# dblanm/gnn-manip

Measured on AMD Instinct MI355X. Metric: rollout steps/sec (N particles, 10 MP steps, hidden=128), higher is better.
Workload: dtype f32; 1 GPU; north_star target: N=100k dense synthetic scene, conn_r=0.015, max_neighbours=20, hidden=128, 10 MP steps; n_particles=100000, hidden=128, edges_last_step=1966056, k_steps=6, candidates_per_gpu=1, parallelism=candidate-parallel x1

## Files before the change

### gnn_manip_amd/csrc/common.h

```cpp
#pragma once
#include <hip/hip_runtime.h>
#include <stdint.h>
#include <stdio.h>
#include <string.h>
#include <mutex>
#include "../../include/gnn_manip_hip.h"

namespace gm {

void set_error(const char* fmt, ...);

#define GM_HIP_CHECK(expr)                                                                  \
    do {                                                                                    \
        hipError_t _e = (expr);                                                             \
        if (_e != hipSuccess) {                                                             \
            gm::set_error("%s failed: %s (%s:%d)", #expr, hipGetErrorString(_e), __FILE__,  \
                          __LINE__);                                                        \
            return GM_ERR_HIP;                                                              \
        }                                                                                   \
    } while (0)

#define GM_REQUIRE(cond, code, ...)          \
    do {                                     \
        if (!(cond)) {                       \
// ... 57 lines not shown
    }
    size_t used() const { return align_up(off, 256); }
};

enum : int { ERRF_NONFINITE_POS = 1, ERRF_BAD_EDGE_INDEX = 2, ERRF_CAPACITY = 4, ERRF_SPLIT_RANGE = 8 };

struct GraphHeader {
    int n_edges;
    int error_flags;
    int ncells;
    int dims[3];
    unsigned bbox_min[3];
    unsigned bbox_max[3];
    double origin[3];
    double inv_h;
    int n_per_graph;
    int ncells_local;
    int ticket;
    int order_skip;
};

struct GraphWs {
    GraphHeader* hdr;
    int* cell_of;
    int* cell_start;
    int* cell_cursor;
    float4* sorted;
    int* cnt;
    int* out_ptr;
    int* nbr;
    int* scan_cells;
    int* scan_cnt;
    int max_cells;
    size_t bytes;
};
int max_cells_for(int64_t n);
GraphWs carve_graph(void* ws, int64_t n, int max_nb);

struct CsrHeader {
    int n_edges;
    int error_flags;
    int flow;
    int pad;
};
struct CsrWs {
    CsrHeader* hdr;
    int* in_ptr;
    int* cursor;
    int* dst;
    int* src;
    int* eid;
    int* scan_in;
    int* sort_tmp;
    int64_t cap;
    int* blocks;
    size_t bytes;
};
CsrWs carve_csr(void* ws, int64_t n, int64_t cap);

enum ProfKind : int { PROF_EDGE = 0, PROF_NODE = 1, PROF_GRAPH = 2, PROF_ENC = 3, PROF_REST = 4, PROF_KINDS = 5 };
constexpr int PROF_MAX = 4096;
struct ProfState {
    int mask = 0;
    int count[PROF_KINDS] = {};
    int dropped[PROF_KINDS] = {};
    hipEvent_t* start[PROF_KINDS] = {};
    hipEvent_t* stop[PROF_KINDS] = {};
    ~ProfState();
};
struct ProfScope {
    ProfState* p;
    int idx;
    int kind;
    hipStream_t s;
    ProfScope(ProfState* state, int kind, hipStream_t s);
    ~ProfScope();
};

struct StepClear;
int rollout_pre_features(float* obs, int64_t n, const gm_feature_desc* d, const int* rank, const float* target, float* out,
                         hipStream_t s, const StepClear* clear);
int rollout_integrate_post(float* obs, int64_t n, const gm_feature_desc* d, const float* pred, const int* rank,
                           const float* target, float* pred_out, hipStream_t s);
int renumber_gather(const float* in, float* out, int k, int64_t n, int D, const int* perm, const void* graph_ws, const int* total_in,
                    int* total_out, const int* rank_caller, int* rank_out, hipStream_t s);
int renumber_scatter(const float* in, float* out, int frames, int64_t n, int D, const int* total, hipStream_t s);
int csr_from_graph_with_features(const void* graph_ws, int64_t n, int K, void* csr_ws, size_t csr_ws_bytes, const float* pos,
                                 int64_t pos_stride, float conn_r, float* edge_attr, int flow, hipStream_t s);
int csr_from_edge_index(const int64_t* ei, int64_t n, int64_t e, int flow, void* csr_ws, size_t csr_ws_bytes, bool with_blocks, hipStream_t stream);

int cell_order(const float* pos, int64_t pos_stride, int64_t n, int64_t n_per, double conn_r, int K, void* graph_ws, size_t graph_ws_bytes,
               int* perm, hipStream_t s);

size_t scan_state_ints(int64_t n_max);
struct ScanJob {
    const int* in;
    int* out;
    long long n;
    int* total_out;
    int* state;
};
int scan_lookback(const ScanJob* jobs, int n_jobs, hipStream_t s);

struct ClearJob {
    int* p;
    long long n;
    int v;
};
constexpr int kClearJobsMax = 12;
struct GraphHeader;
struct StepClear {
    int n_jobs = 0;
    ClearJob job[kClearJobsMax] = {};
    GraphHeader* gh = nullptr;
    CsrHeader* ch = nullptr;
    int flow = 0;
    int add(int* p, long long n, int v) {
        if (!p || n <= 0) return GM_OK;
        GM_REQUIRE(n_jobs < kClearJobsMax, GM_ERR_INVALID_ARGUMENT, "StepClear: more than %d resets in one pass", kClearJobsMax);
        job[n_jobs++] = ClearJob{p, n, v};
        return GM_OK;
    }
};
int launch_step_clear(const StepClear& c, hipStream_t s);
#if defined(__HIPCC__)
__device__ inline void step_clear_run(const StepClear& c, long long t, long long nt) {
    for (int q = 0; q < c.n_jobs; ++q) {
        int* p = c.job[q].p;
        const long long n = c.job[q].n;
        const int v = c.job[q].v;
        if ((reinterpret_cast<uintptr_t>(p) & 15) == 0 && n >= 4) {
            const long long n4 = n >> 2;
            int4* p4 = reinterpret_cast<int4*>(p);
            for (long long i = t; i < n4; i += nt) p4[i] = make_int4(v, v, v, v);
            for (long long i = (n4 << 2) + t; i < n; i += nt) p[i] = v;
        } else {
            for (long long i = t; i < n; i += nt) p[i] = v;
        }
    }
    if (t == 0) {
        if (GraphHeader* hdr = c.gh) {
            hdr->n_edges = 0;
            hdr->error_flags = 0;
            hdr->ncells = 1;
            for (int a = 0; a < 3; ++a) {
                hdr->bbox_min[a] = 0xffffffffu;
                hdr->bbox_max[a] = 0u;
                hdr->dims[a] = 1;
                hdr->origin[a] = 0.0;
            }
            hdr->inv_h = 1.0;
            hdr->n_per_graph = 1;
            hdr->ncells_local = 1;
            hdr->ticket = 0;
            hdr->order_skip = 0;
        }
        if (CsrHeader* ch = c.ch) {
            ch->n_edges = 0;
            ch->error_flags = 0;
            ch->flow = c.flow;
            ch->pad = 0;
        }
    }
}
#endif
struct GraphWs;
// ... 11 lines not shown
```

### gnn_manip_amd/csrc/features.hip

```cpp
#include "common.h"

namespace gm {

struct FeatParams {
    int k, D, cart, mat, ctrl;
    float r;
    float vm[3], vs[3], am[3], as[3], lo[3], hi[3];
};

static int to_params(const gm_feature_desc* d, FeatParams* p, const char* who) {
    GM_REQUIRE(d != nullptr, GM_ERR_INVALID_ARGUMENT, "%s: null feature descriptor", who);
    GM_REQUIRE(d->k_steps >= 2 && d->k_steps <= 64, GM_ERR_INVALID_ARGUMENT, "%s: k_steps=%d out of range", who, d->k_steps);
    GM_REQUIRE(d->data_dim >= 4 && d->cart_col >= 0 && d->cart_col + 3 <= d->data_dim, GM_ERR_INVALID_ARGUMENT,
               "%s: bad cartesian columns", who);
    GM_REQUIRE(d->material_col >= 0 && d->material_col < d->data_dim, GM_ERR_INVALID_ARGUMENT, "%s: bad material column", who);
    GM_REQUIRE(d->control_col < 0 || d->control_col + 3 <= d->data_dim, GM_ERR_INVALID_ARGUMENT, "%s: bad control columns", who);
    GM_REQUIRE(d->conn_r > 0.0, GM_ERR_INVALID_ARGUMENT, "%s: conn_r must be > 0", who);
    p->k = d->k_steps; p->D = d->data_dim; p->cart = d->cart_col; p->mat = d->material_col; p->ctrl = d->control_col;
    p->r = (float)d->conn_r;
    for (int a = 0; a < 3; ++a) {
        p->vm[a] = d->vel_mean[a]; p->vs[a] = d->vel_std[a];
        p->am[a] = d->acc_mean[a]; p->as[a] = d->acc_std[a];
        p->lo[a] = d->lower_bounds[a]; p->hi[a] = d->upper_bounds[a];
    }
// ... 1 lines not shown
}

__global__ void __launch_bounds__(256) node_features_kernel(const float* __restrict__ obs, int64_t n, FeatParams P,
                                                             float* __restrict__ out) {
    const int64_t i = (int64_t)blockIdx.x * blockDim.x + threadIdx.x;
    if (i >= n) return;
    const int F = 3 * (P.k - 1) + 7 + (P.ctrl >= 0 ? 3 : 0);
    float* o = out + i * F;
    const int64_t fs = n * P.D;
    const float* row = obs + i * P.D;
    float prev[3], cur[3];
#pragma unroll
    for (int a = 0; a < 3; ++a) prev[a] = row[P.cart + a];
    for (int t = 1; t < P.k; ++t) {
#pragma unroll
        for (int a = 0; a < 3; ++a) {
            cur[a] = row[t * fs + P.cart + a];
            o[(t - 1) * 3 + a] = __fdiv_rn(__fsub_rn(__fsub_rn(cur[a], prev[a]), P.vm[a]), P.vs[a]);
            prev[a] = cur[a];
        }
    }
    float* b = o + 3 * (P.k - 1);
#pragma unroll
    for (int a = 0; a < 3; ++a) {
        float l = __fdiv_rn(__fsub_rn(cur[a], P.lo[a]), P.r);
        float u = __fdiv_rn(__fsub_rn(P.hi[a], cur[a]), P.r);
        b[a] = fminf(fmaxf(l, -1.f), 1.f);
        b[3 + a] = fminf(fmaxf(u, -1.f), 1.f);
    }
    const float* last = row + (int64_t)(P.k - 1) * fs;
    b[6] = last[P.mat];
    if (P.ctrl >= 0) {
#pragma unroll
        for (int a = 0; a < 3; ++a) b[7 + a] = __fdiv_rn(__fsub_rn(last[P.ctrl + a], P.vm[a]), P.vs[a]);
    }
}

__device__ __forceinline__ void edge_feat(const float* __restrict__ pos, int64_t stride, int64_t s, int64_t r, float cr,
                                          float* __restrict__ o) {
    float d[3];
#pragma unroll
    for (int a = 0; a < 3; ++a) d[a] = __fdiv_rn(__fsub_rn(pos[s * stride + a], pos[r * stride + a]), cr);
    float q = __fmul_rn(d[0], d[0]);
    q = __fadd_rn(q, __fmul_rn(d[1], d[1]));
    q = __fadd_rn(q, __fmul_rn(d[2], d[2]));
    *reinterpret_cast<float4*>(o) = make_float4(d[0], d[1], d[2], __fsqrt_rn(q));
}

__global__ void __launch_bounds__(256) edge_features_kernel(const float* __restrict__ pos, int64_t stride,
                                                             const int64_t* __restrict__ snd,
                                                             const int64_t* __restrict__ rcv, int64_t e, float cr,
                                                             float* __restrict__ out) {
    const int64_t i = (int64_t)blockIdx.x * blockDim.x + threadIdx.x;
    if (i >= e) return;
    edge_feat(pos, stride, snd[i], rcv[i], cr, out + i * 4);
}

__global__ void __launch_bounds__(256) edge_features_csr_kernel(const float* __restrict__ pos, int64_t stride,
                                                                 const CsrHeader* __restrict__ hdr,
                                                                 const int* __restrict__ src, const int* __restrict__ dst,
                                                                 float cr, float* __restrict__ out) {
    const int e = hdr->n_edges;
    const bool swap = hdr->flow != 0;
    for (int64_t i = (int64_t)blockIdx.x * blockDim.x + threadIdx.x; i < e; i += (int64_t)gridDim.x * blockDim.x)
        edge_feat(pos, stride, swap ? dst[i] : src[i], swap ? src[i] : dst[i], cr, out + i * 4);
}

__global__ void __launch_bounds__(256) integrate_kernel(const float* __restrict__ pred, const float* __restrict__ obs,
                                                         int64_t n, FeatParams P, float* __restrict__ next_pos) {
    const int64_t i = (int64_t)blockIdx.x * blockDim.x + threadIdx.x;
    if (i >= n) return;
    const int64_t fs = n * P.D;
    const float* l1 = obs + (int64_t)(P.k - 1) * fs + i * P.D + P.cart;
    const float* l2 = obs + (int64_t)(P.k - 2) * fs + i * P.D + P.cart;
#pragma unroll
    for (int a = 0; a < 3; ++a) {
        float acc = __fadd_rn(__fmul_rn(pred[i * 3 + a], P.as[a]), P.am[a]);
        float lv = __fsub_rn(l1[a], l2[a]);
        float v = __fadd_rn(lv, acc);
        next_pos[i * 3 + a] = __fadd_rn(l1[a], v);
    }
}

__global__ void __launch_bounds__(256) pre_features_kernel(float* __restrict__ obs, int64_t n, FeatParams P,
                                                            const int* __restrict__ rank, const float* __restrict__ target,
                                                            float* __restrict__ out, StepClear clr) {
    const int64_t i = (int64_t)blockIdx.x * blockDim.x + threadIdx.x;
    step_clear_run(clr, i, (long long)gridDim.x * blockDim.x);
    if (i >= n) return;
    const int64_t fs = n * P.D;
    float* row = obs + i * P.D;
    float* last = row + (int64_t)(P.k - 1) * fs;
    if (rank && P.ctrl >= 0) {
        const int rk = rank[i];
        if (rk >= 0) {
#pragma unroll
            for (int a = 0; a < 3; ++a) {
                const float cur = last[P.cart + a];
                last[P.ctrl + a] = target ? __fsub_rn(target[(int64_t)rk * 3 + a], cur) : cur;
            }
        }
    }
    const int F = 3 * (P.k - 1) + 7 + (P.ctrl >= 0 ? 3 : 0);
    float* o = out + i * F;
    float prev[3], cur[3];
#pragma unroll
    for (int a = 0; a < 3; ++a) prev[a] = row[P.cart + a];
    for (int t = 1; t < P.k; ++t) {
#pragma unroll
        for (int a = 0; a < 3; ++a) {
            cur[a] = row[t * fs + P.cart + a];
            o[(t - 1) * 3 + a] = __fdiv_rn(__fsub_rn(__fsub_rn(cur[a], prev[a]), P.vm[a]), P.vs[a]);
            prev[a] = cur[a];
        }
    }
    float* b = o + 3 * (P.k - 1);
#pragma unroll
    for (int a = 0; a < 3; ++a) {
        float l = __fdiv_rn(__fsub_rn(cur[a], P.lo[a]), P.r);
        float u = __fdiv_rn(__fsub_rn(P.hi[a], cur[a]), P.r);
        b[a] = fminf(fmaxf(l, -1.f), 1.f);
        b[3 + a] = fminf(fmaxf(u, -1.f), 1.f);
    }
    b[6] = last[P.mat];
    if (P.ctrl >= 0) {
#pragma unroll
        for (int a = 0; a < 3; ++a) b[7 + a] = __fdiv_rn(__fsub_rn(last[P.ctrl + a], P.vm[a]), P.vs[a]);
    }
}

__global__ void __launch_bounds__(256) integrate_post_kernel(float* __restrict__ obs, int64_t n, FeatParams P,
                                                              const float* __restrict__ pred, const int* __restrict__ rank,
                                                              const float* __restrict__ target, float* __restrict__ pred_out) {
    const int64_t i = (int64_t)blockIdx.x * blockDim.x + threadIdx.x;
    if (i >= n) return;
    const int64_t fs = n * P.D;
    float* row = obs + i * P.D;
    const float* l1 = row + (int64_t)(P.k - 1) * fs + P.cart;
    const float* l2 = row + (int64_t)(P.k - 2) * fs + P.cart;
    float nxt[3];
#pragma unroll
    for (int a = 0; a < 3; ++a) {
        const float pa = pred[i * 3 + a];
        if (pred_out) pred_out[i * 3 + a] = pa;
        const float acc = __fadd_rn(__fmul_rn(pa, P.as[a]), P.am[a]);
        const float lv = __fsub_rn(l1[a], l2[a]);
        nxt[a] = __fadd_rn(l1[a], __fadd_rn(lv, acc));
    }
    for (int t = 0; t + 1 < P.k; ++t)
        for (int d = 0; d < P.D; ++d) row[t * fs + d] = row[(t + 1) * fs + d];
    float* last = row + (int64_t)(P.k - 1) * fs;
    const int rk = rank ? rank[i] : -1;
    if (rk < 0) {
#pragma unroll
        for (int a = 0; a < 3; ++a) last[P.cart + a] = nxt[a];
    } else if (target) {
#pragma unroll
        for (int a = 0; a < 3; ++a) last[P.cart + a] = target[(int64_t)rk * 3 + a];
    }
}

__global__ void __launch_bounds__(1024) rigid_rank_kernel(const float* __restrict__ obs, int64_t n, FeatParams P,
                                                           int* __restrict__ rank, int* __restrict__ n_rigid) {
    __shared__ int wsum[16];
    __shared__ int carry_s;
    const float* last = obs + (int64_t)(P.k - 1) * n * P.D;
    const int lane = threadIdx.x & 63, wave = threadIdx.x >> 6;
    if (threadIdx.x == 0) carry_s = 0;
    __syncthreads();
    for (int64_t b = 0; b < n; b += 1024) {
        int64_t i = b + threadIdx.x;
        int f = (i < n && last[i * P.D + P.mat] == 1.0f) ? 1 : 0;
        int incl = f;
#pragma unroll
        for (int d = 1; d < 64; d <<= 1) {
            int t = __shfl_up(incl, d, 64);
            if (lane >= d) incl += t;
        }
        if (lane == 63) wsum[wave] = incl;
        __syncthreads();
        int base = carry_s;
        for (int w = 0; w < wave; ++w) base += wsum[w];
        if (i < n) rank[i] = f ? base + incl - 1 : -1;
        __syncthreads();
        if (threadIdx.x == 1023) carry_s = base + incl;
        __syncthreads();
    }
    if (threadIdx.x == 0 && n_rigid) *n_rigid = carry_s;
}

__global__ void __launch_bounds__(256) state_pre_kernel(float* __restrict__ obs, int64_t n, FeatParams P,
                                                         const int* __restrict__ rank, const float* __restrict__ target) {
    const int64_t i = (int64_t)blockIdx.x * blockDim.x + threadIdx.x;
    if (i >= n) return;
    const int rk = rank[i];
    if (rk < 0) return;
    float* last = obs + (int64_t)(P.k - 1) * n * P.D + i * P.D;
#pragma unroll
    for (int a = 0; a < 3; ++a) {
        float cur = last[P.cart + a];
        last[P.ctrl + a] = target ? __fsub_rn(target[(int64_t)rk * 3 + a], cur) : cur;
    }
}

__global__ void __launch_bounds__(256) state_post_kernel(float* __restrict__ obs, int64_t n, FeatParams P,
                                                          const float* __restrict__ next_pos,
                                                          const int* __restrict__ rank, const float* __restrict__ target) {
    const int64_t i = (int64_t)blockIdx.x * blockDim.x + threadIdx.x;
    if (i >= n) return;
    const int64_t fs = n * P.D;
    float* row = obs + i * P.D;
    for (int t = 0; t + 1 < P.k; ++t)
        for (int d = 0; d < P.D; ++d) row[t * fs + d] = row[(t + 1) * fs + d];
    float* last = row + (int64_t)(P.k - 1) * fs;
    const int rk = rank ? rank[i] : -1;
    if (rk < 0) {
#pragma unroll
        for (int a = 0; a < 3; ++a) last[P.cart + a] = next_pos[i * 3 + a];
    } else if (target) {
#pragma unroll
        for (int a = 0; a < 3; ++a) last[P.cart + a] = target[(int64_t)rk * 3 + a];
    }
}

__global__ void __launch_bounds__(256) rigid_transform_kernel(const float* __restrict__ init, int64_t nr,
                                                               const float* __restrict__ cst, int64_t steps, float tx,
                                                               float ty, float tz, float* __restrict__ out) {
    const int64_t id = (int64_t)blockIdx.x * blockDim.x + threadIdx.x;
    if (id >= nr * steps) return;
    const int64_t t = id / nr, i = id - t * nr;
    const float c = cst[t * 3], s = cst[t * 3 + 1], typ = cst[t * 3 + 2];
    const float i0 = __fsub_rn(tx, init[i * 3 + 0]);
    const float i1 = __fsub_rn(ty, init[i * 3 + 2]);
    const float i2 = __fsub_rn(tz, init[i * 3 + 1]);
    const float p0 = __fadd_rn(i0, tx);
    const float p1 = __fadd_rn(__fmaf_rn(-s, i2, __fmul_rn(c, i1)), typ);
    const float p2 = __fadd_rn(__fmaf_rn(c, i2, __fmul_rn(s, i1)), tz);
    out[id * 3 + 0] = p0;
    out[id * 3 + 2] = p1;
    out[id * 3 + 1] = p2;
}

// ... 5 lines not shown
    const float* gt = g + t * nr * 3;
    double dc = 0.0, ds = 0.0, dt = 0.0;
    for (int64_t i = tid; i < nr; i += 256) {
        const double i1 = (double)ty - (double)init[i * 3 + 2];
        const double i2 = (double)tz - (double)init[i * 3 + 1];
        const double g1 = gt[i * 3 + 1], g2 = gt[i * 3 + 2];
        dc += g2 * i1 + g1 * i2;
        ds += g1 * i1 - g2 * i2;
        dt += g2;
    }
    red[0][tid] = dc; red[1][tid] = ds; red[2][tid] = dt;
    __syncthreads();
    for (int w = 128; w >= 1; w >>= 1) {
        if (tid < w) {
#pragma unroll
            for (int a = 0; a < 3; ++a) red[a][tid] += red[a][tid + w];
        }
        __syncthreads();
    }
    if (tid < 3) d_cst[t * 3 + tid] = (float)red[tid][0];
}

__global__ void __launch_bounds__(256) renumber_gather_kernel(const float* __restrict__ in, float* __restrict__ out, int k, int64_t n, int D,
                                                               const int* __restrict__ perm, const GraphHeader* __restrict__ ghdr,
                                                               const int* __restrict__ total_in, int* __restrict__ total_out,
                                                               const int* __restrict__ rank_caller, int* __restrict__ rank_out) {
    const int64_t id = (int64_t)blockIdx.x * blockDim.x + threadIdx.x;
    if (id >= (int64_t)k * n) return;
    const int64_t t = id / n, j = id - t * n;
    const int64_t src = ghdr->order_skip ? j : (int64_t)perm[j];
    const float* a = in + (t * n + src) * D;
    float* b = out + (t * n + j) * D;
    for (int d = 0; d < D; ++d) b[d] = a[d];
    if (t == 0) {
        const int tot = total_in ? total_in[src] : (int)src;
        total_out[j] = tot;
        if (rank_out) rank_out[j] = rank_caller[tot];
    }
}
__global__ void __launch_bounds__(256) renumber_scatter_kernel(const float* __restrict__ in, float* __restrict__ out, int frames, int64_t n, int D,
                                                                const int* __restrict__ total) {
    const int64_t id = (int64_t)blockIdx.x * blockDim.x + threadIdx.x;
    if (id >= (int64_t)frames * n) return;
    const int64_t t = id / n, j = id - t * n;
    const float* a = in + (t * n + j) * D;
    float* b = out + (t * n + (int64_t)total[j]) * D;
    for (int d = 0; d < D; ++d) b[d] = a[d];
}
int renumber_gather(const float* in, float* out, int k, int64_t n, int D, const int* perm, const void* graph_ws, const int* total_in,
                    int* total_out, const int* rank_caller, int* rank_out, hipStream_t s) {
    if (n <= 0 || k <= 0) return GM_OK;
    hipLaunchKernelGGL(renumber_gather_kernel, dim3((unsigned)cdiv((int64_t)k * n, 256)), dim3(256), 0, s, in, out, k, n, D, perm,
                       static_cast<const GraphHeader*>(graph_ws), total_in, total_out, rank_caller, rank_out);
    GM_LAUNCH_CHECK();
    return GM_OK;
}
int renumber_scatter(const float* in, float* out, int frames, int64_t n, int D, const int* total, hipStream_t s) {
    if (n <= 0 || frames <= 0) return GM_OK;
    hipLaunchKernelGGL(renumber_scatter_kernel, dim3((unsigned)cdiv((int64_t)frames * n, 256)), dim3(256), 0, s, in, out, frames, n, D, total);
    GM_LAUNCH_CHECK();
    return GM_OK;
}

int rollout_pre_features(float* obs, int64_t n, const gm_feature_desc* d, const int* rank, const float* target, float* out,
                         hipStream_t s, const StepClear* clear) {
    FeatParams P;
    int rc = to_params(d, &P, "gm_rollout_step");
    if (rc != GM_OK) return rc;
    hipLaunchKernelGGL(pre_features_kernel, dim3((unsigned)cdiv(n, 256)), dim3(256), 0, s, obs, n, P, rank, target, out, clear ? *clear : StepClear{});
    GM_LAUNCH_CHECK();
    return GM_OK;
}

int rollout_integrate_post(float* obs, int64_t n, const gm_feature_desc* d, const float* pred, const int* rank,
                           const float* target, float* pred_out, hipStream_t s) {
    FeatParams P;
    int rc = to_params(d, &P, "gm_rollout_step");
    if (rc != GM_OK) return rc;
    hipLaunchKernelGGL(integrate_post_kernel, dim3((unsigned)cdiv(n, 256)), dim3(256), 0, s, obs, n, P, pred, rank, target, pred_out);
    GM_LAUNCH_CHECK();
    return GM_OK;
}



__global__ void __launch_bounds__(256) node_features_bwd_kernel(const float* __restrict__ obs, int64_t n, FeatParams P,
                                                                 const float* __restrict__ g, float* __restrict__ d_obs) {
    const int64_t i = (int64_t)blockIdx.x * blockDim.x + threadIdx.x;
    if (i >= n) return;
    const int F = 3 * (P.k - 1) + 7 + (P.ctrl >= 0 ? 3 : 0);
    const float* gi = g + i * F;
    const int64_t fs = n * P.D;
    float* row = d_obs + i * P.D;
    for (int t = 0; t < P.k; ++t)
        for (int d = 0; d < P.D; ++d) row[t * fs + d] = 0.f;
    for (int t = 0; t < P.k; ++t) {
#pragma unroll
        for (int a = 0; a < 3; ++a) {
            float v = 0.f;
            if (t >= 1) v = __fdiv_rn(gi[(t - 1) * 3 + a], P.vs[a]);
            if (t + 1 < P.k) v = __fsub_rn(v, __fdiv_rn(gi[t * 3 + a], P.vs[a]));
            row[t * fs + P.cart + a] = v;
        }
    }
    const float* b = gi + 3 * (P.k - 1);
    const float* last_in = obs + (int64_t)(P.k - 1) * fs + i * P.D;
    float* last = row + (int64_t)(P.k - 1) * fs;
#pragma unroll
    for (int a = 0; a < 3; ++a) {
        const float cur = last_in[P.cart + a];
        const float l = __fdiv_rn(__fsub_rn(cur, P.lo[a]), P.r);
        const float u = __fdiv_rn(__fsub_rn(P.hi[a], cur), P.r);
        float v = last[P.cart + a];
        if (l >= -1.f && l <= 1.f) v = __fadd_rn(v, __fdiv_rn(b[a], P.r));
        if (u >= -1.f && u <= 1.f) v = __fsub_rn(v, __fdiv_rn(b[3 + a], P.r));
        last[P.cart + a] = v;
    }
    if (P.ctrl >= 0) {
#pragma unroll
        for (int a = 0; a < 3; ++a) last[P.ctrl + a] = __fdiv_rn(b[7 + a], P.vs[a]);
    }
}

__global__ void __launch_bounds__(256) integrate_bwd_kernel(const float* __restrict__ g, int64_t n, FeatParams P,
                                                             float* __restrict__ d_pred, float* __restrict__ d_obs) {
    const int64_t i = (int64_t)blockIdx.x * blockDim.x + threadIdx.x;
    if (i >= n) return;
    const int64_t fs = n * P.D;
    float* row = d_obs + i * P.D;
    for (int t = 0; t < P.k; ++t)
        for (int d = 0; d < P.D; ++d) row[t * fs + d] = 0.f;
#pragma unroll
    for (int a = 0; a < 3; ++a) {
        const float ga = g[i * 3 + a];
        d_pred[i * 3 + a] = __fmul_rn(ga, P.as[a]);
        row[(int64_t)(P.k - 1) * fs + P.cart + a] = __fmul_rn(2.f, ga);
        row[(int64_t)(P.k - 2) * fs + P.cart + a] = -ga;
    }
}

__device__ __forceinline__ void state_pre_bwd_row(float* __restrict__ last, const FeatParams& P, bool has_target, float* __restrict__ gt,
                                                  const float* __restrict__ post_t) {
#pragma unroll
    for (int a = 0; a < 3; ++a) {
        const float gc = last[P.ctrl + a];
        const float gx = last[P.cart + a];
        last[P.cart + a] = has_target ? __fsub_rn(gx, gc) : __fadd_rn(gx, gc);
        last[P.ctrl + a] = 0.f;
        if (gt) gt[a] = has_target ? (post_t ? __fadd_rn(post_t[a], gc) : gc) : 0.f;
    }
}

__global__ void __launch_bounds__(256) state_pre_bwd_kernel(const float* __restrict__ d_after, int64_t n, FeatParams P,
                                                             const int* __restrict__ rank, int has_target, float* __restrict__ d_before,
                                                             float* __restrict__ d_target) {
    const int64_t i = (int64_t)blockIdx.x * blockDim.x + threadIdx.x;
    if (i >= n) return;
    const int64_t fs = n * P.D;
    const float* in = d_after + i * P.D;
    float* row = d_before + i * P.D;
    for (int t = 0; t < P.k; ++t)
        for (int d = 0; d < P.D; ++d) row[t * fs + d] = in[t * fs + d];
    const int rk = rank[i];
    if (rk >= 0) state_pre_bwd_row(row + (int64_t)(P.k - 1) * fs, P, has_target != 0, d_target ? d_target + (int64_t)rk * 3 : nullptr, nullptr);
}

// ... 362 lines not shown
```

### gnn_manip_amd/csrc/graph.hip

```cpp
#include <stdarg.h>
#include "common.h"
#include "hedge.h"
#include "blocks_dev.h"

namespace gm {

static thread_local char g_err[512] = "";
void set_error(const char* fmt, ...) {
    va_list ap;
    va_start(ap, fmt);
    vsnprintf(g_err, sizeof(g_err), fmt, ap);
    va_end(ap);
}
const char* last_error() { return g_err; }

ProfState::~ProfState() {
    for (int k = 0; k < PROF_KINDS; ++k) {
        if (!start[k]) continue;
        for (int i = 0; i < PROF_MAX; ++i) { (void)hipEventDestroy(start[k][i]); (void)hipEventDestroy(stop[k][i]); }
        delete[] start[k];
        delete[] stop[k];
    }
}

// ... 285 lines not shown
        ext[a] = mx - mn;
    }
    double h = r * (1.0 + 1.0 / 1024.0);
    if (!(h > 0.0)) h = 1.0;
    int d[3];
    for (;;) {
        double prod = 1.0;
        for (int a = 0; a < 3; ++a) {
            double c = floor(ext[a] / h) + 1.0;
            if (c > 2.0e9) c = 2.0e9;
            d[a] = (int)c;
            prod *= c;
        }
        if (prod <= (double)max_cells) break;
        h *= 1.2599210498948732;
    }
    for (int a = 0; a < 3; ++a) {
        hdr->dims[a] = d[a];
        hdr->origin[a] = lo[a];
    }
    hdr->inv_h = 1.0 / h;
    hdr->ncells_local = d[0] * d[1] * d[2];
    hdr->ncells = hdr->ncells_local * (int)n_graphs;
    hdr->n_per_graph = (int)(n_per > 0 ? n_per : (n > 0 ? n : 1));
}

__device__ __forceinline__ int cell_coord(float v, double origin, double inv_h, int dim) {
    double c = floor(((double)v - origin) * inv_h);
    int ci = (c > 0.0) ? (c < (double)(dim - 1) ? (int)c : dim - 1) : 0;
    return ci;
}

__global__ void __launch_bounds__(256) cell_assign_kernel(const float* __restrict__ pos, int64_t stride, int64_t n,
                                                           const GraphHeader* __restrict__ hdr,
                                                           int* __restrict__ cell_of, int* __restrict__ cell_count) {
    int64_t i = (int64_t)blockIdx.x * blockDim.x + threadIdx.x;
    if (i >= n) return;
    const int dx = hdr->dims[0], dy = hdr->dims[1], dz = hdr->dims[2];
    float x = pos[i * stride], y = pos[i * stride + 1], z = pos[i * stride + 2];
    if (!isfinite(x)) x = 0.f;
    if (!isfinite(y)) y = 0.f;
    if (!isfinite(z)) z = 0.f;
    int cx = cell_coord(x, hdr->origin[0], hdr->inv_h, dx);
    int cy = cell_coord(y, hdr->origin[1], hdr->inv_h, dy);
    int cz = cell_coord(z, hdr->origin[2], hdr->inv_h, dz);
    int c = (int)(i / hdr->n_per_graph) * hdr->ncells_local + (cz * dy + cy) * dx + cx;
    cell_of[i] = c;
    atomicAdd(&cell_count[c], 1);
}

__global__ void __launch_bounds__(256) cell_fill_kernel(const float* __restrict__ pos, int64_t stride, int64_t n,
                                                         const int* __restrict__ cell_of,
                                                         const int* __restrict__ cell_start,
                                                         int* __restrict__ cell_cursor, float4* __restrict__ sorted) {
    int64_t i = (int64_t)blockIdx.x * blockDim.x + threadIdx.x;
    if (i >= n) return;
    int c = cell_of[i];
    int p = cell_start[c] + atomicAdd(&cell_cursor[c], 1);
    sorted[p] = make_float4(pos[i * stride], pos[i * stride + 1], pos[i * stride + 2], __int_as_float((int)i));
}

constexpr int kCellOrderCap = 1024;
__global__ void __launch_bounds__(256) cell_order_kernel(const float4* __restrict__ sorted, const int* __restrict__ cell_of,
                                                          const int* __restrict__ cell_start, GraphHeader* hdr, int64_t n,
                                                          int* __restrict__ perm) {
    const int64_t p = (int64_t)blockIdx.x * blockDim.x + threadIdx.x;
    if (p >= n) return;
    const int i = __float_as_int(sorted[p].w);
    const int c = cell_of[i];
    const int lo = cell_start[c], hi = cell_start[c + 1];
    if (hi - lo > kCellOrderCap) {
        if (p == lo) atomicOr(&hdr->order_skip, 1);
        return;
    }
    int before = 0;
    for (int q = lo; q < hi; ++q) before += __float_as_int(sorted[q].w) < i ? 1 : 0;
    perm[lo + before] = i;
}

constexpr int NB_LPQ = 16;
constexpr int NB_CAP = 96;
constexpr int NB_STRIDE = NB_CAP + 1;
constexpr int NB_QPB = 256 / NB_LPQ;

__global__ void __launch_bounds__(256) neighbor_fast_kernel(const float4* __restrict__ sorted,
                                                             const int* __restrict__ cell_start,
                                                             const GraphHeader* __restrict__ hdr, int64_t n, double r2,
                                                             int K, int* __restrict__ cnt, int* __restrict__ nbr,
                                                             int* __restrict__ indeg, int* __restrict__ arrival, int flow) {
    __shared__ double sd2[NB_QPB * NB_STRIDE];
    __shared__ int sj[NB_QPB * NB_STRIDE];
    const int tid = threadIdx.x, sub = tid & (NB_LPQ - 1), ql = tid / NB_LPQ, lane = tid & 63;
    const int grp_shift = (lane / NB_LPQ) * NB_LPQ;
    const int64_t slot = (int64_t)blockIdx.x * NB_QPB + ql;
    const bool active = slot < n;
    const float4 q = sorted[active ? slot : 0];
    const int qi = __float_as_int(q.w);
    const int dx = hdr->dims[0], dy = hdr->dims[1], dz = hdr->dims[2];
    const double inv_h = hdr->inv_h;
    const int cx = cell_coord(q.x, hdr->origin[0], inv_h, dx);
    const int cy = cell_coord(q.y, hdr->origin[1], inv_h, dy);
    const int cz = cell_coord(q.z, hdr->origin[2], inv_h, dz);
    const double qx = (double)q.x, qy = (double)q.y, qz = (double)q.z;
    const int cbase = (qi / hdr->n_per_graph) * hdr->ncells_local;
    double* ld = sd2 + ql * NB_STRIDE;
    int* lj = sj + ql * NB_STRIDE;
    int count = 0;
    const int x0 = max(cx - 1, 0), x1 = min(cx + 1, dx - 1);
    if (active) {
        for (int z = max(cz - 1, 0); z <= min(cz + 1, dz - 1); ++z) {
            for (int y = max(cy - 1, 0); y <= min(cy + 1, dy - 1); ++y) {
                const int row = cbase + (z * dy + y) * dx;
                const int b = cell_start[row + x0], e = cell_start[row + x1 + 1];
                for (int c0 = b; c0 < e; c0 += NB_LPQ) {
                    const int c = c0 + sub;
                    bool in = false;
                    double d2 = 0.0;
                    int j = 0;
                    if (c < e) {
                        const float4 p = sorted[c];
                        double d = qx - (double)p.x;
                        d2 = __dmul_rn(d, d);
                        d = qy - (double)p.y;
                        d2 = __dadd_rn(d2, __dmul_rn(d, d));
                        d = qz - (double)p.z;
                        d2 = __dadd_rn(d2, __dmul_rn(d, d));
                        in = d2 <= r2;
                        j = __float_as_int(p.w);
                    }
                    const unsigned m = (unsigned)(__ballot(in) >> grp_shift) & ((1u << NB_LPQ) - 1u);
                    const int pos = count + __popc(m & ((1u << sub) - 1u));
                    if (in && pos < NB_CAP) {
                        ld[pos] = d2;
                        lj[pos] = j;
                    }
                    count += __popc(m);
                }
            }
        }
    }
    __syncthreads();
    if (!active) return;
    if (count > NB_CAP) {
        if (sub == 0) cnt[qi] = -1;
        return;
    }
    for (int a0 = sub; a0 < count; a0 += 4 * NB_LPQ) {
        double da[4];
        int ja[4], rank[4];
#pragma unroll
        for (int u = 0; u < 4; ++u) {
            const int a = a0 + NB_LPQ * u;
            da[u] = a < count ? ld[a] : -1.0;
            ja[u] = a < count ? lj[a] : 0;
            rank[u] = 0;
        }
        for (int f = 0; f < count; ++f) {
            const double df = ld[f];
            const int jf = lj[f];
#pragma unroll
            for (int u = 0; u < 4; ++u) rank[u] += (df < da[u] || (df == da[u] && jf < ja[u])) ? 1 : 0;
        }
#pragma unroll
        for (int u = 0; u < 4; ++u)
            if (a0 + NB_LPQ * u < count && rank[u] < K) {
                nbr[(int64_t)qi * K + rank[u]] = ja[u];
                if (indeg) arrival[(int64_t)qi * K + rank[u]] = atomicAdd(&indeg[flow ? qi : ja[u]], 1);
            }
    }
    if (sub == 0) cnt[qi] = count < K ? count : K;
}

template <int BS>
__global__ void __launch_bounds__(BS) neighbor_kernel(const float4* __restrict__ sorted,
                                                       const int* __restrict__ cell_start,
                                                       const GraphHeader* __restrict__ hdr, int64_t n, double r2,
                                                       int K, int* __restrict__ cnt, int* __restrict__ nbr,
                                                       int* __restrict__ indeg, int* __restrict__ arrival, int flow) {
    extern __shared__ __attribute__((aligned(16))) char smem[];
    double* kd = reinterpret_cast<double*>(smem);
    int* ki = reinterpret_cast<int*>(smem + (size_t)K * BS * 8);
    const int t = threadIdx.x;
    const int64_t slot = (int64_t)blockIdx.x * BS + t;
    if (slot >= n) return;
    const float4 q = sorted[slot];
    const int qi = __float_as_int(q.w);
    if (cnt[qi] != -1) return;
    const int cbase = (qi / hdr->n_per_graph) * hdr->ncells_local;
    const int dx = hdr->dims[0], dy = hdr->dims[1], dz = hdr->dims[2];
    const double inv_h = hdr->inv_h;
    const int cx = cell_coord(q.x, hdr->origin[0], inv_h, dx);
    const int cy = cell_coord(q.y, hdr->origin[1], inv_h, dy);
    const int cz = cell_coord(q.z, hdr->origin[2], inv_h, dz);
    const double qx = (double)q.x, qy = (double)q.y, qz = (double)q.z;
    int kept = 0;
    const int x0 = max(cx - 1, 0), x1 = min(cx + 1, dx - 1);
    for (int z = max(cz - 1, 0); z <= min(cz + 1, dz - 1); ++z) {
        for (int y = max(cy - 1, 0); y <= min(cy + 1, dy - 1); ++y) {
            const int row = cbase + (z * dy + y) * dx;
            const int b = cell_start[row + x0], e = cell_start[row + x1 + 1];
            for (int c = b; c < e; ++c) {
                const float4 p = sorted[c];
                double d = qx - (double)p.x;
                double d2 = __dmul_rn(d, d);
                d = qy - (double)p.y;
                d2 = __dadd_rn(d2, __dmul_rn(d, d));
                d = qz - (double)p.z;
                d2 = __dadd_rn(d2, __dmul_rn(d, d));
                if (!(d2 <= r2)) continue;
                const int j = __float_as_int(p.w);
                int pos;
                if (kept < K) {
                    pos = kept++;
                } else {
                    const double ld = kd[(K - 1) * BS + t];
                    const int lj = ki[(K - 1) * BS + t];
                    if (!(d2 < ld || (d2 == ld && j < lj))) continue;
                    pos = K - 1;
                }
                while (pos > 0) {
                    const double pd = kd[(pos - 1) * BS + t];
// ... 470 lines not shown
```

### gnn_manip_amd/csrc/model.hip

```cpp
#include <algorithm>
#include <vector>
#include "common.h"
#include "mlp.h"
#include "model.h"
#include "train.h"
#include "hedge.h"
#include "hmlp.h"

using namespace gm;

std::vector<MlpSpec> gm::model_mlps(const gm_model_desc& d) {
    const int H = d.hidden_size, NL = d.num_layers;
    std::vector<MlpSpec> mlp;
    auto add = [&](int in, int out, bool normed) {
        const int base = mlp.empty() ? 0 : mlp.back().end;
        mlp.push_back({base, base + 2 * (NL + 1) + (normed ? 2 : 0), in, out, normed});
    };
    add(d.edge_dim, H, true);
    add(d.node_dim, H, true);
    for (int k = 0; k < d.m_steps; ++k) {
        add(3 * H, H, true);
        add(2 * H, H, true);
    }
    add(H, d.out_dim, false);
// ... 586 lines not shown
    r.bytes = c.used();
    return r;
}
struct RenumberWs {
    float* state[2];
    int* total[2];
    int *perm, *rank;
    size_t bytes;
};
RenumberWs carve_renumber(void* ws, const gm_feature_desc* fd, int64_t n) {
    RenumberWs w;
    Carver c(ws);
    const size_t st = (size_t)fd->k_steps * n * fd->data_dim;
    w.state[0] = c.take<float>(st);
    w.state[1] = c.take<float>(st);
    w.total[0] = c.take<int>(n);
    w.total[1] = c.take<int>(n);
    w.perm = c.take<int>(n);
    w.rank = c.take<int>(n);
    w.bytes = c.used();
    return w;
}
}

extern "C" {

int gm_model_set_edge_kernel(gm_model* m, int choice) {
    GM_REQUIRE(m, GM_ERR_INVALID_ARGUMENT, "gm_model_set_edge_kernel: null model");
    GM_REQUIRE(choice >= EK_AUTO && choice <= EK_SYS_ALL, GM_ERR_INVALID_ARGUMENT, "gm_model_set_edge_kernel: choice %d out of range", choice);
    GM_REQUIRE(choice == EK_AUTO || choice >= EK_SYS, GM_ERR_UNSUPPORTED,
               "gm_model_set_edge_kernel: choices 1..4 (the round-1 fp32 / bf16 x 6 kernels) were removed from the library (round 5)");
    GM_REQUIRE((choice != EK_SYS && choice != EK_SYS_ALL) || m->packed_h3, GM_ERR_UNSUPPORTED, "gm_model_set_edge_kernel: the systolic kernel is for hidden_size 128, num_layers 2");
    m->edge_kernel = choice;
    return GM_OK;
}

int gm_model_set_node_fusion(gm_model* m, int on) {
    GM_REQUIRE(m, GM_ERR_INVALID_ARGUMENT, "gm_model_set_node_fusion: null model");
    m->node_fusion = on != 0;
    return GM_OK;
}

int gm_model_set_precision(gm_model* m, int precision) {
    GM_REQUIRE(m, GM_ERR_INVALID_ARGUMENT, "gm_model_set_precision: null model");
    GM_REQUIRE(precision == GM_PRECISION_F32 || precision == GM_PRECISION_F16, GM_ERR_INVALID_ARGUMENT,
               "gm_model_set_precision: precision %d (GM_PRECISION_F32 = 0, GM_PRECISION_F16 = 1)", precision);
    m->precision = precision;
    return GM_OK;
}

int gm_model_profile(gm_model* m, int kind_mask) {
    GM_REQUIRE(m, GM_ERR_INVALID_ARGUMENT, "gm_model_profile: null model");
    if (!m->prof) {
        if (!kind_mask) return GM_OK;
        m->prof = new ProfState();
    }
    for (int k = 0; k < PROF_KINDS; ++k)
        if (((kind_mask & ~m->prof->mask) >> k) & 1) m->prof->count[k] = m->prof->dropped[k] = 0;
    m->prof->mask = kind_mask;
    return GM_OK;
}

int gm_model_profile_query(const gm_model* m, int kind, int64_t* launches, double* total_ms) {
    GM_REQUIRE(m && kind >= 0 && kind < PROF_KINDS && launches && total_ms, GM_ERR_INVALID_ARGUMENT, "gm_model_profile_query: bad argument");
    *launches = 0;
    *total_ms = 0.0;
    const ProfState* p = m->prof;
    if (!p) return GM_OK;
    *launches = p->dropped[kind] ? -(int64_t)(p->count[kind] + p->dropped[kind]) : p->count[kind];
    for (int i = 0; i < p->count[kind]; ++i) {
        GM_HIP_CHECK(hipEventSynchronize(p->stop[kind][i]));
        float ms = 0.f;
        GM_HIP_CHECK(hipEventElapsedTime(&ms, p->start[kind][i], p->stop[kind][i]));
        *total_ms += ms;
    }
    return GM_OK;
}

size_t gm_rollout_workspace_bytes(const gm_model_desc* desc, int64_t n, int K) {
    if (!desc || n < 0 || K < 1) return 0;
    return carve_rollout(nullptr, desc, n, K).bytes;
}

int gm_rollout_step(const gm_model* m, float* obs, int64_t n, const gm_feature_desc* fd, int K, const int32_t* rigid_rank,
                    const float* rigid_target, float* pred_acc_out, void* ws, size_t ws_bytes, void* stream) {
    gm::DevGuard dev_guard(obs);
    GM_REQUIRE(m && obs && fd && ws, GM_ERR_INVALID_ARGUMENT, "gm_rollout_step: null pointer");
    const int F = 3 * (fd->k_steps - 1) + 7 + (fd->control_col >= 0 ? 3 : 0);
    GM_REQUIRE(m->d.node_dim == F, GM_ERR_INVALID_ARGUMENT, "gm_rollout_step: model node_dim=%d but features give %d", m->d.node_dim, F);
    GM_REQUIRE(m->d.edge_dim == 4 && m->d.out_dim == 3, GM_ERR_INVALID_ARGUMENT, "gm_rollout_step: needs edge_dim=4, out_dim=3 (3-D scene)");
    GM_REQUIRE(n < ((int64_t)1 << 31) / (K > 0 ? K : 1), GM_ERR_UNSUPPORTED, "gm_rollout_step: n*max_neighbours overflows int32");
    RolloutWs r = carve_rollout(ws, &m->d, n, K);
    GM_REQUIRE(ws_bytes >= r.bytes, GM_ERR_WORKSPACE, "gm_rollout_step: workspace %zu < %zu", ws_bytes, r.bytes);
    if (n == 0) return GM_OK;
    const int64_t cap = n * K;
    int rc;
    hipStream_t hs = (hipStream_t)stream;
    {
        StepClear clr;
        rc = graph_clear_jobs(clr, carve_graph(r.graph, n, K), n);
        if (rc == GM_OK) rc = csr_clear_jobs(clr, carve_csr(r.csr, n, cap), n, m->d.flow);
        FwdWs f = carve_fwd(r.fwd, m->Hp, n, cap, cap);
        if (rc == GM_OK) rc = clr.add(reinterpret_cast<int*>(f.agg), (long long)n * m->Hp, 0);
        if (rc != GM_OK) return rc;
        ProfScope prof(m->prof, PROF_REST, hs);
        rc = gm::rollout_pre_features(obs, n, fd, rigid_rank, rigid_target, r.x, hs, &clr);
    }
    if (rc != GM_OK) return rc;
    const float* last_pos = obs + (size_t)(fd->k_steps - 1) * n * fd->data_dim + fd->cart_col;
    {
        ProfScope prof(m->prof, PROF_GRAPH, hs);
        rc = gm::radius_graph_build_fused(last_pos, fd->data_dim, n, fd->nodes_per_graph > 0 ? fd->nodes_per_graph : n, fd->conn_r, K,
                                          r.graph, r.graph_bytes, r.csr, r.csr_bytes, m->d.flow, hs);
    }
    if (rc != GM_OK) return rc;
    {
        ProfScope prof(m->prof, PROF_REST, hs);
        rc = gm::csr_from_graph_fused(r.graph, n, K, r.csr, r.csr_bytes, last_pos, fd->data_dim, (float)fd->conn_r, r.edge_attr,
                                      m->d.flow, hs);
    }
    if (rc != GM_OK) return rc;
    rc = epd_forward_impl(m, r.x, n, r.edge_attr, 1, r.csr, cap, r.pred, r.fwd, r.fwd_bytes, stream, true,
                          fd->nodes_per_graph > 0 ? fd->nodes_per_graph : n);
    if (rc != GM_OK) return rc;
    ProfScope prof(m->prof, PROF_REST, hs);
    return gm::rollout_integrate_post(obs, n, fd, r.pred, rigid_rank, rigid_target, pred_acc_out, hs);
}

size_t gm_rollout_renumber_workspace_bytes(const gm_feature_desc* fd, int64_t n) {
    if (!fd || n < 0 || fd->k_steps < 1 || fd->data_dim < 1) return 0;
    return carve_renumber(nullptr, fd, n).bytes;
}

int gm_rollout(const gm_model* m, float* obs, int64_t n, const gm_feature_desc* fd, int K, const int32_t* rigid_rank,
               const float* rigid_targets, int64_t n_targets, int64_t n_rigid, int64_t steps, float* record_last,
               int64_t renumber_every, void* renumber_ws, size_t renumber_ws_bytes, void* ws, size_t ws_bytes, void* stream) {
    gm::DevGuard dev_guard(obs);
    GM_REQUIRE(m && obs && fd && ws, GM_ERR_INVALID_ARGUMENT, "gm_rollout: null pointer");
    GM_REQUIRE(steps >= 0 && n_targets >= 0 && n_rigid >= 0 && renumber_every >= 0, GM_ERR_INVALID_ARGUMENT, "gm_rollout: negative count");
    GM_REQUIRE(rigid_targets || n_targets == 0 || n_rigid == 0, GM_ERR_INVALID_ARGUMENT, "gm_rollout: n_targets > 0 without rigid_targets");
    GM_REQUIRE(!rigid_targets || rigid_rank, GM_ERR_INVALID_ARGUMENT, "gm_rollout: rigid_targets need rigid_rank");
    hipStream_t hs = (hipStream_t)stream;
    const size_t frame = (size_t)n * fd->data_dim;
    const bool renum = renumber_every > 0 && n > 0 && steps > 0;
    RenumberWs rw{};
    RolloutWs r{};
    if (renum) {
        GM_REQUIRE(renumber_ws, GM_ERR_INVALID_ARGUMENT, "gm_rollout: renumber_every > 0 needs renumber_ws (gm_rollout_renumber_workspace_bytes)");
        rw = carve_renumber(renumber_ws, fd, n);
        GM_REQUIRE(renumber_ws_bytes >= rw.bytes, GM_ERR_WORKSPACE, "gm_rollout: renumber workspace %zu < %zu", renumber_ws_bytes, rw.bytes);
        GM_REQUIRE(n < ((int64_t)1 << 31) / (K > 0 ? K : 1), GM_ERR_UNSUPPORTED, "gm_rollout: n*max_neighbours overflows int32");
        r = carve_rollout(ws, &m->d, n, K);
        GM_REQUIRE(ws_bytes >= r.bytes, GM_ERR_WORKSPACE, "gm_rollout: workspace %zu < %zu", ws_bytes, r.bytes);
    }
    float* state = obs;
    const int* rank = rigid_rank;
    const int* total = nullptr;
    int flip = 0;
    for (int64_t i = 0; i < steps; ++i) {
        if (renum && i % renumber_every == 0) {
            const float* last_pos = state + (size_t)(fd->k_steps - 1) * frame + fd->cart_col;
            int rc = gm::cell_order(last_pos, fd->data_dim, n, fd->nodes_per_graph > 0 ? fd->nodes_per_graph : n, fd->conn_r, K, r.graph,
                                    r.graph_bytes, rw.perm, hs);
            if (rc != GM_OK) return rc;
            rc = gm::renumber_gather(state, rw.state[flip], fd->k_steps, n, fd->data_dim, rw.perm, r.graph, total, rw.total[flip],
                                     rigid_rank, rigid_rank ? rw.rank : nullptr, hs);
            if (rc != GM_OK) return rc;
            state = rw.state[flip];
            total = rw.total[flip];
            rank = rigid_rank ? rw.rank : nullptr;
            flip ^= 1;
        }
        float* last = state + (size_t)(fd->k_steps - 1) * frame;
        const float* target = i < n_targets ? rigid_targets + (size_t)i * n_rigid * 3 : nullptr;
        if (record_last) {
            int rc = fd->control_col >= 0 ? gm_state_pre(state, n, fd, rank, target, stream) : GM_OK;
            if (rc != GM_OK) return rc;
            if (total) rc = gm::renumber_scatter(last, record_last + (size_t)i * frame, 1, n, fd->data_dim, total, hs);
            else GM_HIP_CHECK(hipMemcpyAsync(record_last + (size_t)i * frame, last, frame * sizeof(float), hipMemcpyDeviceToDevice, hs));
            if (rc != GM_OK) return rc;
        }
        int rc = gm_rollout_step(m, state, n, fd, K, rank, target, nullptr, ws, ws_bytes, stream);
        if (rc != GM_OK) return rc;
    }
    if (total) return gm::renumber_scatter(state, obs, fd->k_steps, n, fd->data_dim, total, hs);
    return GM_OK;
}

int gm_rollout_status(const void* ws, const gm_model_desc* desc, int64_t n, int K, int64_t* n_edges_host, void* stream) {
    gm::DevGuard dev_guard(ws);
    GM_REQUIRE(ws && desc && n_edges_host, GM_ERR_INVALID_ARGUMENT, "gm_rollout_status: null pointer");
    RolloutWs r = carve_rollout(const_cast<void*>(ws), desc, n, K);
    int rc = gm_radius_graph_num_edges(r.graph, n_edges_host, stream);
    if (rc != GM_OK) return rc;
    int64_t e2 = 0;
    return gm_csr_num_edges(r.csr, &e2, stream);
}

}
```

Before: 126.8 rollout steps/s.

## Fuse step-boundary integrate/pre-features kernels and prefetch neighbour cell runs

In the rollout loop, the integrate-post of one step and the pre-features of the next step are merged into a single step_boundary kernel that also runs the workspace clears. This removes a kernel launch and a separate pass over the observation buffer per step. The neighbour search kernel now assigns one of the 9 cell-row runs to each lane and prefetches the first candidate of six runs ahead, reducing load latency stalls. The change adds control-flow complexity and more registers in the neighbour kernel, and it touches out-of-range slot 0 for empty runs.

```diff
diff --git a/gnn_manip_amd/csrc/common.h b/gnn_manip_amd/csrc/common.h
--- a/gnn_manip_amd/csrc/common.h
+++ b/gnn_manip_amd/csrc/common.h
@@ -163,6 +163,8 @@
                          hipStream_t s, const StepClear* clear);
 int rollout_integrate_post(float* obs, int64_t n, const gm_feature_desc* d, const float* pred, const int* rank,
                            const float* target, float* pred_out, hipStream_t s);
+int rollout_step_boundary(float* obs, int64_t n, const gm_feature_desc* d, const float* pred, const int* rank, const float* target_post,
+                          const float* target_pre, float* out, hipStream_t s, const StepClear* clear);
 int renumber_gather(const float* in, float* out, int k, int64_t n, int D, const int* perm, const void* graph_ws, const int* total_in,
                     int* total_out, const int* rank_caller, int* rank_out, hipStream_t s);
 int renumber_scatter(const float* in, float* out, int frames, int64_t n, int D, const int* total, hipStream_t s);
diff --git a/gnn_manip_amd/csrc/features.hip b/gnn_manip_amd/csrc/features.hip
--- a/gnn_manip_amd/csrc/features.hip
+++ b/gnn_manip_amd/csrc/features.hip
@@ -107,12 +107,8 @@
     }
 }
 
-__global__ void __launch_bounds__(256) pre_features_kernel(float* __restrict__ obs, int64_t n, FeatParams P,
-                                                            const int* __restrict__ rank, const float* __restrict__ target,
-                                                            float* __restrict__ out, StepClear clr) {
-    const int64_t i = (int64_t)blockIdx.x * blockDim.x + threadIdx.x;
-    step_clear_run(clr, i, (long long)gridDim.x * blockDim.x);
-    if (i >= n) return;
+__device__ __forceinline__ void pre_features_row(float* __restrict__ obs, int64_t n, const FeatParams& P, const int* __restrict__ rank,
+                                                 const float* __restrict__ target, float* __restrict__ out, int64_t i) {
     const int64_t fs = n * P.D;
     float* row = obs + i * P.D;
     float* last = row + (int64_t)(P.k - 1) * fs;
@@ -153,12 +149,18 @@
         for (int a = 0; a < 3; ++a) b[7 + a] = __fdiv_rn(__fsub_rn(last[P.ctrl + a], P.vm[a]), P.vs[a]);
     }
 }
-
-__global__ void __launch_bounds__(256) integrate_post_kernel(float* __restrict__ obs, int64_t n, FeatParams P,
-                                                              const float* __restrict__ pred, const int* __restrict__ rank,
-                                                              const float* __restrict__ target, float* __restrict__ pred_out) {
-    const int64_t i = (int64_t)blockIdx.x * blockDim.x + threadIdx.x;
-    if (i >= n) return;
+__global__ void __launch_bounds__(256) pre_features_kernel(float* __restrict__ obs, int64_t n, FeatParams P,
+                                                            const int* __restrict__ rank, const float* __restrict__ target,
+                                                            float* __restrict__ out, StepClear clr) {
+    const int64_t i = (int64_t)blockIdx.x * blockDim.x + threadIdx.x;
+    step_clear_run(clr, i, (long long)gridDim.x * blockDim.x);
+    if (i >= n) return;
+    pre_features_row(obs, n, P, rank, target, out, i);
+}
+
+__device__ __forceinline__ void integrate_post_row(float* __restrict__ obs, int64_t n, const FeatParams& P, const float* __restrict__ pred,
+                                                   const int* __restrict__ rank, const float* __restrict__ target,
+                                                   float* __restrict__ pred_out, int64_t i) {
     const int64_t fs = n * P.D;
     float* row = obs + i * P.D;
     const float* l1 = row + (int64_t)(P.k - 1) * fs + P.cart;
@@ -183,6 +185,24 @@
 #pragma unroll
         for (int a = 0; a < 3; ++a) last[P.cart + a] = target[(int64_t)rk * 3 + a];
     }
+}
+__global__ void __launch_bounds__(256) integrate_post_kernel(float* __restrict__ obs, int64_t n, FeatParams P,
+                                                              const float* __restrict__ pred, const int* __restrict__ rank,
+                                                              const float* __restrict__ target, float* __restrict__ pred_out) {
+    const int64_t i = (int64_t)blockIdx.x * blockDim.x + threadIdx.x;
+    if (i >= n) return;
+    integrate_post_row(obs, n, P, pred, rank, target, pred_out, i);
+}
+
+__global__ void __launch_bounds__(256) step_boundary_kernel(float* __restrict__ obs, int64_t n, FeatParams P,
+                                                             const float* __restrict__ pred, const int* __restrict__ rank,
+                                                             const float* __restrict__ target_post, const float* __restrict__ target_pre,
+                                                             float* __restrict__ out, StepClear clr) {
+    const int64_t i = (int64_t)blockIdx.x * blockDim.x + threadIdx.x;
+    step_clear_run(clr, i, (long long)gridDim.x * blockDim.x);
+    if (i >= n) return;
+    integrate_post_row(obs, n, P, pred, rank, target_post, nullptr, i);
+    pre_features_row(obs, n, P, rank, target_pre, out, i);
 }
 
 __global__ void __launch_bounds__(1024) rigid_rank_kernel(const float* __restrict__ obs, int64_t n, FeatParams P,
@@ -354,6 +374,16 @@
     return GM_OK;
 }
 
+int rollout_step_boundary(float* obs, int64_t n, const gm_feature_desc* d, const float* pred, const int* rank, const float* target_post,
+                          const float* target_pre, float* out, hipStream_t s, const StepClear* clear) {
+    FeatParams P;
+    int rc = to_params(d, &P, "gm_rollout");
+    if (rc != GM_OK) return rc;
+    hipLaunchKernelGGL(step_boundary_kernel, dim3((unsigned)cdiv(n, 256)), dim3(256), 0, s, obs, n, P, pred, rank, target_post, target_pre,
+                       out, clear ? *clear : StepClear{});
+    GM_LAUNCH_CHECK();
+    return GM_OK;
+}
 
 
 __global__ void __launch_bounds__(256) node_features_bwd_kernel(const float* __restrict__ obs, int64_t n, FeatParams P,
diff --git a/gnn_manip_amd/csrc/graph.hip b/gnn_manip_amd/csrc/graph.hip
--- a/gnn_manip_amd/csrc/graph.hip
+++ b/gnn_manip_amd/csrc/graph.hip
@@ -391,6 +391,8 @@
 constexpr int NB_CAP = 96;
 constexpr int NB_STRIDE = NB_CAP + 1;
 constexpr int NB_QPB = 256 / NB_LPQ;
+constexpr int NB_RUNS = 9;
+constexpr int NB_PF = 6;
 
 __global__ void __launch_bounds__(256) neighbor_fast_kernel(const float4* __restrict__ sorted,
                                                              const int* __restrict__ cell_start,
@@ -416,36 +418,49 @@
     int* lj = sj + ql * NB_STRIDE;
     int count = 0;
     const int x0 = max(cx - 1, 0), x1 = min(cx + 1, dx - 1);
-    if (active) {
-        for (int z = max(cz - 1, 0); z <= min(cz + 1, dz - 1); ++z) {
-            for (int y = max(cy - 1, 0); y <= min(cy + 1, dy - 1); ++y) {
-                const int row = cbase + (z * dy + y) * dx;
-                const int b = cell_start[row + x0], e = cell_start[row + x1 + 1];
-                for (int c0 = b; c0 < e; c0 += NB_LPQ) {
-                    const int c = c0 + sub;
-                    bool in = false;
-                    double d2 = 0.0;
-                    int j = 0;
-                    if (c < e) {
-                        const float4 p = sorted[c];
-                        double d = qx - (double)p.x;
-                        d2 = __dmul_rn(d, d);
-                        d = qy - (double)p.y;
-                        d2 = __dadd_rn(d2, __dmul_rn(d, d));
-                        d = qz - (double)p.z;
-                        d2 = __dadd_rn(d2, __dmul_rn(d, d));
-                        in = d2 <= r2;
-                        j = __float_as_int(p.w);
-                    }
-                    const unsigned m = (unsigned)(__ballot(in) >> grp_shift) & ((1u << NB_LPQ) - 1u);
-                    const int pos = count + __popc(m & ((1u << sub) - 1u));
-                    if (in && pos < NB_CAP) {
-                        ld[pos] = d2;
-                        lj[pos] = j;
-                    }
-                    count += __popc(m);
-                }
+    int rb, re;
+    {
+        const int rz = cz - 1 + sub / 3, ry = cy - 1 + sub % 3;
+        const bool ok = active && sub < NB_RUNS && rz >= 0 && rz < dz && ry >= 0 && ry < dy;
+        const int row = cbase + (min(max(rz, 0), dz - 1) * dy + min(max(ry, 0), dy - 1)) * dx;
+        const int b = cell_start[row + x0], e = cell_start[row + x1 + 1];
+        rb = ok ? b : 0;
+        re = ok ? e : 0;
+    }
+    auto first = [&](int u) {
+        const int c = __shfl(rb, u, NB_LPQ) + sub;
+        return sorted[c < __shfl(re, u, NB_LPQ) ? c : 0];
+    };
+    float4 pf[NB_PF];
+#pragma unroll
+    for (int u = 0; u < NB_PF; ++u) pf[u] = first(u);
+#pragma unroll
+    for (int u = 0; u < NB_RUNS; ++u) {
+        const int b = __shfl(rb, u, NB_LPQ), e = __shfl(re, u, NB_LPQ);
+        float4 p = pf[u % NB_PF];
+        if (u + NB_PF < NB_RUNS) pf[u % NB_PF] = first(u + NB_PF);
+        for (int c0 = b;;) {
+            bool in = false;
+            double d2 = 0.0;
+            if (c0 + sub < e) {
+                double d = qx - (double)p.x;
+                d2 = __dmul_rn(d, d);
+                d = qy - (double)p.y;
+                d2 = __dadd_rn(d2, __dmul_rn(d, d));
+                d = qz - (double)p.z;
+                d2 = __dadd_rn(d2, __dmul_rn(d, d));
+                in = d2 <= r2;
             }
+            const unsigned m = (unsigned)(__ballot(in) >> grp_shift) & ((1u << NB_LPQ) - 1u);
+            const int pos = count + __popc(m & ((1u << sub) - 1u));
+            if (in && pos < NB_CAP) {
+                ld[pos] = d2;
+                lj[pos] = __float_as_int(p.w);
+            }
+            count += __popc(m);
+            c0 += NB_LPQ;
+            if (c0 >= e) break;
+            if (c0 + sub < e) p = sorted[c0 + sub];
         }
     }
     __syncthreads();
diff --git a/gnn_manip_amd/csrc/model.hip b/gnn_manip_amd/csrc/model.hip
--- a/gnn_manip_amd/csrc/model.hip
+++ b/gnn_manip_amd/csrc/model.hip
@@ -692,31 +692,39 @@
     return carve_rollout(nullptr, desc, n, K).bytes;
 }
 
-int gm_rollout_step(const gm_model* m, float* obs, int64_t n, const gm_feature_desc* fd, int K, const int32_t* rigid_rank,
-                    const float* rigid_target, float* pred_acc_out, void* ws, size_t ws_bytes, void* stream) {
-    gm::DevGuard dev_guard(obs);
+}
+
+namespace {
+int step_check(const gm_model* m, const float* obs, int64_t n, const gm_feature_desc* fd, int K, void* ws, size_t ws_bytes, RolloutWs* r) {
     GM_REQUIRE(m && obs && fd && ws, GM_ERR_INVALID_ARGUMENT, "gm_rollout_step: null pointer");
     const int F = 3 * (fd->k_steps - 1) + 7 + (fd->control_col >= 0 ? 3 : 0);
     GM_REQUIRE(m->d.node_dim == F, GM_ERR_INVALID_ARGUMENT, "gm_rollout_step: model node_dim=%d but features give %d", m->d.node_dim, F);
     GM_REQUIRE(m->d.edge_dim == 4 && m->d.out_dim == 3, GM_ERR_INVALID_ARGUMENT, "gm_rollout_step: needs edge_dim=4, out_dim=3 (3-D scene)");
     GM_REQUIRE(n < ((int64_t)1 << 31) / (K > 0 ? K : 1), GM_ERR_UNSUPPORTED, "gm_rollout_step: n*max_neighbours overflows int32");
-    RolloutWs r = carve_rollout(ws, &m->d, n, K);
-    GM_REQUIRE(ws_bytes >= r.bytes, GM_ERR_WORKSPACE, "gm_rollout_step: workspace %zu < %zu", ws_bytes, r.bytes);
-    if (n == 0) return GM_OK;
+    *r = carve_rollout(ws, &m->d, n, K);
+    GM_REQUIRE(ws_bytes >= r->bytes, GM_ERR_WORKSPACE, "gm_rollout_step: workspace %zu < %zu", ws_bytes, r->bytes);
+    return GM_OK;
+}
+int step_clear_jobs(const gm_model* m, const RolloutWs& r, int64_t n, int K, StepClear& clr) {
+    const int64_t cap = n * K;
+    int rc = graph_clear_jobs(clr, carve_graph(r.graph, n, K), n);
+    if (rc == GM_OK) rc = csr_clear_jobs(clr, carve_csr(r.csr, n, cap), n, m->d.flow);
+    FwdWs f = carve_fwd(r.fwd, m->Hp, n, cap, cap);
+    if (rc == GM_OK) rc = clr.add(reinterpret_cast<int*>(f.agg), (long long)n * m->Hp, 0);
+    return rc;
+}
+int step_pre(const gm_model* m, float* obs, int64_t n, const gm_feature_desc* fd, int K, const int32_t* rigid_rank,
+             const float* rigid_target, const RolloutWs& r, hipStream_t hs) {
+    StepClear clr;
+    int rc = step_clear_jobs(m, r, n, K, clr);
+    if (rc != GM_OK) return rc;
+    ProfScope prof(m->prof, PROF_REST, hs);
+    return gm::rollout_pre_features(obs, n, fd, rigid_rank, rigid_target, r.x, hs, &clr);
+}
+int step_graph_forward(const gm_model* m, const float* obs, int64_t n, const gm_feature_desc* fd, int K, const RolloutWs& r, void* stream) {
     const int64_t cap = n * K;
     int rc;
     hipStream_t hs = (hipStream_t)stream;
-    {
-        StepClear clr;
-        rc = graph_clear_jobs(clr, carve_graph(r.graph, n, K), n);
-        if (rc == GM_OK) rc = csr_clear_jobs(clr, carve_csr(r.csr, n, cap), n, m->d.flow);
-        FwdWs f = carve_fwd(r.fwd, m->Hp, n, cap, cap);
-        if (rc == GM_OK) rc = clr.add(reinterpret_cast<int*>(f.agg), (long long)n * m->Hp, 0);
-        if (rc != GM_OK) return rc;
-        ProfScope prof(m->prof, PROF_REST, hs);
-        rc = gm::rollout_pre_features(obs, n, fd, rigid_rank, rigid_target, r.x, hs, &clr);
-    }
-    if (rc != GM_OK) return rc;
     const float* last_pos = obs + (size_t)(fd->k_steps - 1) * n * fd->data_dim + fd->cart_col;
     {
         ProfScope prof(m->prof, PROF_GRAPH, hs);
@@ -730,8 +738,24 @@
                                       m->d.flow, hs);
     }
     if (rc != GM_OK) return rc;
-    rc = epd_forward_impl(m, r.x, n, r.edge_attr, 1, r.csr, cap, r.pred, r.fwd, r.fwd_bytes, stream, true,
-                          fd->nodes_per_graph > 0 ? fd->nodes_per_graph : n);
+    return epd_forward_impl(m, r.x, n, r.edge_attr, 1, r.csr, cap, r.pred, r.fwd, r.fwd_bytes, stream, true,
+                            fd->nodes_per_graph > 0 ? fd->nodes_per_graph : n);
+}
+}
+
+extern "C" {
+
+int gm_rollout_step(const gm_model* m, float* obs, int64_t n, const gm_feature_desc* fd, int K, const int32_t* rigid_rank,
+                    const float* rigid_target, float* pred_acc_out, void* ws, size_t ws_bytes, void* stream) {
+    gm::DevGuard dev_guard(obs);
+    RolloutWs r;
+    int rc = step_check(m, obs, n, fd, K, ws, ws_bytes, &r);
+    if (rc != GM_OK) return rc;
+    if (n == 0) return GM_OK;
+    hipStream_t hs = (hipStream_t)stream;
+    rc = step_pre(m, obs, n, fd, K, rigid_rank, rigid_target, r, hs);
+    if (rc != GM_OK) return rc;
+    rc = step_graph_forward(m, obs, n, fd, K, r, stream);
     if (rc != GM_OK) return rc;
     ProfScope prof(m->prof, PROF_REST, hs);
     return gm::rollout_integrate_post(obs, n, fd, r.pred, rigid_rank, rigid_target, pred_acc_out, hs);
@@ -767,6 +791,7 @@
     const int* rank = rigid_rank;
     const int* total = nullptr;
     int flip = 0;
+    bool pre_done = false;
     for (int64_t i = 0; i < steps; ++i) {
         if (renum && i % renumber_every == 0) {
             const float* last_pos = state + (size_t)(fd->k_steps - 1) * frame + fd->cart_col;
@@ -790,7 +815,23 @@
             else GM_HIP_CHECK(hipMemcpyAsync(record_last + (size_t)i * frame, last, frame * sizeof(float), hipMemcpyDeviceToDevice, hs));
             if (rc != GM_OK) return rc;
         }
-        int rc = gm_rollout_step(m, state, n, fd, K, rank, target, nullptr, ws, ws_bytes, stream);
+        int rc = step_check(m, state, n, fd, K, ws, ws_bytes, &r);
+        if (rc != GM_OK) return rc;
+        if (n == 0) continue;
+        if (!pre_done) rc = step_pre(m, state, n, fd, K, rank, target, r, hs);
+        else { ProfScope prof(m->prof, PROF_REST, hs); }
+        if (rc == GM_OK) rc = step_graph_forward(m, state, n, fd, K, r, stream);
+        if (rc != GM_OK) return rc;
+        pre_done = i + 1 < steps && !record_last && !(renum && (i + 1) % renumber_every == 0);
+        ProfScope prof(m->prof, PROF_REST, hs);
+        if (pre_done) {
+            const float* target_next = i + 1 < n_targets ? rigid_targets + (size_t)(i + 1) * n_rigid * 3 : nullptr;
+            StepClear clr;
+            rc = step_clear_jobs(m, r, n, K, clr);
+            if (rc == GM_OK) rc = gm::rollout_step_boundary(state, n, fd, r.pred, rank, target, target_next, r.x, hs, &clr);
+        } else {
+            rc = gm::rollout_integrate_post(state, n, fd, r.pred, rank, target, nullptr, hs);
+        }
         if (rc != GM_OK) return rc;
     }
     if (total) return gm::renumber_scatter(state, obs, fd->k_steps, n, fd->data_dim, total, hs);
```

Result: no change. 126.6 rollout steps/s (-0.1%).
